# tatsy/normalizing-flows-pytorch

Hardware: AMD Instinct MI355X
Metric: samples/sec (train step: forward flow + log-det + NLL + backward + Adam) (higher is better)
Workload: dtype f32; 1 GPU; Glow CIFAR-shape (3,32,32) L=3 K=32 batch 64 per GPU (512 over 8); per_gpu_batch=64, global_batch=64, parallelism=dp1, hipgraph=True, deterministic=True, dp_one_graph=False

## Files before the change

### normalizing-flows-pytorch_amd/csrc/conv_chain.hip

```cpp
#include <cstdlib>
#include <cstring>
#include <mutex>
#include <unordered_set>
#include "nf_conv_core.h"
#include "nf_det.h"

NF_DET_STATE(nf_ccd)
NF_DET_HOST_API(nf_ccd)
#include "nf_bf16x3.h"
#include "nf_small_plu.h"

#define NF_CC_NL 6
#define NF_CC_NB 5
#define NF_CC_MAX_BLOCKS NF_CONVNET_MAX_BLOCKS

#define NF_CC_WG_SLOTS (NF_CC_NB * NF_CC_MAX_BLOCKS * 64)
#define NF_CC_GROUP 16
#define NF_CC_MAX_GROUPS ((NF_CC_MAX_BLOCKS + NF_CC_GROUP - 1) / NF_CC_GROUP)
#define NF_CC_FLAT_MAX 128
#define NF_CC_STAT_SLOTS (NF_CC_WG_SLOTS + NF_CC_NB * NF_CC_MAX_GROUPS * 64)
static_assert(2 * NF_CC_STAT_SLOTS == NF_CONVNET_WS_FLOATS, "exchange workspace size in include/nfhip.h");

NF_PERSIST_STATE(nf_cc)
NF_PERSIST_HOST_API(nf_cc)
// ... 828 lines not shown
        for (int j = 0; j < 4; ++j) sc[j] = An[64 + min(16 * rt + 4 * lk + j, C - 1)];
        f32x4 acc = (f32x4){0.f, 0.f, 0.f, 0.f};
#pragma unroll
        for (int q = 0; q < KQ; ++q) {
            const int c = 4 * q + lk;
            const float bv = c < C ? gv[q] : 0.f;
            const float a = (ra < C && c < C) ? av[q] : 0.f;
            acc = __builtin_amdgcn_mfma_f32_16x16x4f32(a, bv, acc, 0, 0, 0);
        }
        float* gxb = gx + b * cs.n_full + p;
        const int row = p >> lgWf, xx = p & (cs.W - 1);
#pragma unroll
        for (int j = 0; j < 4; ++j) {
            const int r = 16 * rt + 4 * lk + j;
            const float v = acc[j] * sc[j];
            if (r < C) gxb[(int64_t)r * P] = v;
            int which, m, sp;
            if (cs.mode == NF_SPLIT_CHANNEL) {
                const int hc = C >> 1, sel = r >= hc ? 1 : 0;
                which = sel ^ cs.odd; m = r - sel * hc; sp = p;
            } else {
                const int k = 4 * r + 2 * (row & 1) + (xx & 1);
                const int qd = (k >= C ? 1 : 0) + (k >= 2 * C ? 1 : 0) + (k >= 3 * C ? 1 : 0);
                const int sel = (qd == 1 || qd == 2) ? 1 : 0;
                which = sel ^ cs.odd; m = sel ? k - C : (qd == 0 ? k : k - 2 * C);
                sp = (row >> 1) * cs.w + (xx >> 1);
            }
            if (r < C && which == 0) G0[m * PXW + sidx * HWh + (sp - sp0)] = v;
        }
    };
#pragma unroll
    for (int u = 0; u < 2; ++u) {
        const int item = wid + u * NF_CV_WAVES;
        if (item < nitem && b0 + (item / RT) / per < B) run(item, R.gv[u]);
    }
#pragma unroll 1
    for (int item = wid + 2 * NF_CV_WAVES; item < nitem; item += NF_CV_WAVES) {
        const int blk = item / RT, sidx = blk / per, rem = blk - sidx * per;
        const int64_t b = b0 + sidx;
        if (b >= B) continue;
        const float* gb = d.hd_g_h + b * cs.n_full + fo_lo * cs.W + (rem << 4) + li;
        float gv[KQ];
#pragma unroll
        for (int q = 0; q < KQ; ++q) {
            const int c = 4 * q + lk;
            gv[q] = gb[(int64_t)(c < C ? c : 0) * P];
        }
        run(item, gv);
    }
    NF_CC_STAMP(104);
    asm volatile("s_waitcnt lgkmcnt(0)\n\ts_barrier" ::: "memory");
}
template <int CT>
__device__ __forceinline__ void nf_cc_head_small_bwd(const nf_convnet_bwd_desc& d, const NfSplit& cs, float* hl, int64_t b0, int nsamp,
                                                     int fo_lo, int fo_hi, int64_t B, int PXW, int HWh, int sp0) {
    const int P = cs.H * cs.W, npx = (fo_hi - fo_lo) * cs.W;
    float* const gx = const_cast<float*>(d.cp_g_y);
    float* const G0 = hl + NF_CC_HD_X1;
    const int lgWf = 31 - __clz(cs.W);
    float G[CT];
    int idx = threadIdx.x;
    auto place = [&](int i, int& sidx, int& p, int64_t& base) {
        sidx = i / npx;
        p = fo_lo * cs.W + (i - sidx * npx);
        base = (b0 + sidx) * cs.n_full + p;
    };
    int sidx = 0, p = 0;
    int64_t base = 0;
    bool ok = idx < nsamp * npx;
    if (ok) {
        place(idx, sidx, p, base);
        ok = b0 + sidx < B;
    }
#pragma unroll
    for (int r = 0; r < CT; ++r) G[r] = ok ? d.hd_g_h[base + (int64_t)r * P] : 0.f;
    float Wm[CT][CT], es[CT];
#pragma unroll
    for (int r = 0; r < CT; ++r)
#pragma unroll
        for (int c = 0; c < CT; ++c) Wm[r][c] = d.hd_W[r * CT + c];
#pragma unroll
    for (int c = 0; c < CT; ++c) es[c] = 1.f / expf(d.hd_ls[c]);
    while (idx < nsamp * npx) {
        if (ok) {
            const int row = p >> lgWf, xx = p & (cs.W - 1);
#pragma unroll
            for (int c = 0; c < CT; ++c) {
                float a = 0.f;
#pragma unroll
                for (int r = 0; r < CT; ++r) a = fmaf(Wm[r][c], G[r], a);
                const float v = a * es[c];
                gx[base + (int64_t)c * P] = v;
                int which, m, sp;
                if (cs.mode == NF_SPLIT_CHANNEL) {
                    const int hc = CT >> 1, sel = c >= hc ? 1 : 0;
                    which = sel ^ cs.odd; m = c - sel * hc; sp = p;
                } else {
                    const int k = 4 * c + 2 * (row & 1) + (xx & 1);
                    const int qd = (k >= CT ? 1 : 0) + (k >= 2 * CT ? 1 : 0) + (k >= 3 * CT ? 1 : 0);
                    const int sel = (qd == 1 || qd == 2) ? 1 : 0;
                    which = sel ^ cs.odd; m = sel ? k - CT : (qd == 0 ? k : k - 2 * CT);
                    sp = (row >> 1) * cs.w + (xx >> 1);
                }
                if (which == 0) G0[m * PXW + sidx * HWh + (sp - sp0)] = v;
            }
        }
        idx += NF_CV_THREADS;
        ok = idx < nsamp * npx;
        if (ok) {
            place(idx, sidx, p, base);
            ok = b0 + sidx < B;
        }
#pragma unroll
        for (int r = 0; r < CT; ++r) G[r] = ok ? d.hd_g_h[base + (int64_t)r * P] : 0.f;
    }
    asm volatile("s_waitcnt lgkmcnt(0)\n\ts_barrier" ::: "memory");
}

template <int NPB, int NKQ, bool HALO, bool CPL, int FWc, int CSc, bool PK>
__global__ void __launch_bounds__(NF_CV_THREADS) k_convnet_chain_fwd(nf_convnet_desc d, NfCvGeo g, int I0, int O_out, int training,
                                                                     float eps, float mom, NfSplit cs) {
    static_assert(NPB * NKQ == NF_CV_WAVES, "sixteen waves");
    constexpr int OWN = 16 / NKQ, PXW = 32 * NPB;
    extern __shared__ __attribute__((aligned(16))) float sm[];
    const int OCB = (O_out + 31) / 32;
    const NfCcLds L = nf_cc_lds<NPB, NKQ>(g.CS, OCB);
    float* Wl = sm + L.WL;
    float* RS = sm + L.RS;
    float* kc = sm + L.KC;
    float* kb = sm + L.KB;
    float* red = sm + L.RED;
    const int CSr = FWc > 0 ? CSc : g.CS;
    const int WPs = L.WPs;
    const int lane = threadIdx.x & 63, wid = threadIdx.x >> 6, c32 = lane & 31, hs = lane >> 5;
    const int pb = wid % NPB, kq = wid / NPB;
    const int64_t Npx = g.B * g.HW;
    const int64_t tile = blockIdx.x;
    const int64_t b0 = (tile * PXW) >> g.lgHW;
    constexpr bool halo = HALO;
    const int y0 = halo ? (int)((tile * PXW) & (g.HW - 1)) >> g.lgW : 0;
    unsigned long long* hslots = halo ? (unsigned long long*)d.ws_zero + NF_CC_STAT_SLOTS : nullptr;
    const int px = pb * 32 + c32;
    const int fpos = nf_cv_frame_of(g, px);
    const int64_t P = tile * PXW + px;
    const bool pv = P < Npx;
    const int64_t b = pv ? P >> g.lgHW : 0;
    const int64_t q = pv ? P & (g.HW - 1) : 0;
    const int npb = nf_cc_valid_px(Npx, tile * PXW + 32 * pb, 32);
    unsigned long long* slots = (unsigned long long*)d.ws_zero;
    const unsigned gbase = 8u * (unsigned)d.ws_gen;

    constexpr bool packed = PK;
    constexpr bool cpl = CPL;
    NF_CC_STAMP(0);
#ifdef NF_CC_NO_HEAD_FWD
    const bool headed = false;
#else
    const bool headed = cpl && d.hd_x != nullptr;
#endif
    const int hf = cs.mode == NF_SPLIT_CHECKER ? 2 : 1;
    const int h_ns = halo ? 1 : (g.HW < PXW ? PXW >> g.lgHW : 1);
    const int h_olo = halo ? hf * y0 : 0, h_ohi = halo ? hf * (y0 + g.TH) : cs.H;
    const int h_rlo = halo ? max(h_olo - hf, 0) : 0, h_rhi = halo ? min(h_ohi + hf, cs.H) : cs.H;
    const int h_per = ((h_rhi - h_rlo) * cs.W) >> 4, h_nblk = h_ns * h_per;
    const int h_sp0 = (h_rlo / hf) * g.W, h_np1 = ((h_rhi - h_rlo) / hf) * g.W;
    const bool hsmall = headed && cs.C <= 4;
    NfCcHeadReq hreq;
    if (headed && !hsmall) {
        if (cs.C <= 16) nf_cc_head_request<4>(hreq, d, cs, b0, h_rlo, h_per, h_nblk, g.B);
        else if (cs.C <= 24) nf_cc_head_request<6>(hreq, d, cs, b0, h_rlo, h_per, h_nblk, g.B);
        else if (cs.C <= 48) nf_cc_head_request<12>(hreq, d, cs, b0, h_rlo, h_per, h_nblk, g.B);
        else nf_cc_head_request<16>(hreq, d, cs, b0, h_rlo, h_per, h_nblk, g.B);
    }
    NF_CC_STAMP(105);
    for (int e = threadIdx.x; e < 3 * NF_CC_FP(g.CS); e += NF_CV_THREADS) sm[L.FA + e] = 0.f;
    float* Fr = sm + L.FA;
    NF_CC_STAMP(106);
    if (hsmall) {
        const bool add_ld = !halo || y0 == 0;
        if (cs.C == 3) nf_cc_head_small_fwd<3>(d, cs, RS, b0, h_ns, h_rlo, h_rhi, h_olo, h_ohi, h_sp0, h_np1, g.B, add_ld);
        else if (cs.C == 4) nf_cc_head_small_fwd<4>(d, cs, RS, b0, h_ns, h_rlo, h_rhi, h_olo, h_ohi, h_sp0, h_np1, g.B, add_ld);
        else nf_cc_head_small_fwd<2>(d, cs, RS, b0, h_ns, h_rlo, h_rhi, h_olo, h_ohi, h_sp0, h_np1, g.B, add_ld);
    } else if (headed) {
        const bool add_ld = !halo || y0 == 0;
        if (cs.C <= 16) nf_cc_head_fwd<4>(hreq, d, cs, RS, b0, h_ns, h_rlo, h_olo, h_ohi, h_per, h_nblk, h_sp0, h_np1, g.B, add_ld);
        else if (cs.C <= 24) nf_cc_head_fwd<6>(hreq, d, cs, RS, b0, h_ns, h_rlo, h_olo, h_ohi, h_per, h_nblk, h_sp0, h_np1, g.B, add_ld);
        else if (cs.C <= 48) nf_cc_head_fwd<12>(hreq, d, cs, RS, b0, h_ns, h_rlo, h_olo, h_ohi, h_per, h_nblk, h_sp0, h_np1, g.B, add_ld);
        else nf_cc_head_fwd<16>(hreq, d, cs, RS, b0, h_ns, h_rlo, h_olo, h_ohi, h_per, h_nblk, h_sp0, h_np1, g.B, add_ld);
    }
    NF_CC_STAMP(107);
    if (cpl && !headed) {
        if (!halo) {
            const int nsamp = g.HW < PXW ? PXW >> g.lgHW : 1;
            const int64_t left = g.B - b0;
            const int n4 = (int)(left < nsamp ? (left > 0 ? left : 0) : nsamp) * (cs.n_full >> 2);
            const float4* src = reinterpret_cast<const float4*>(d.cp_z + b0 * cs.n_full);
            float4* dst = reinterpret_cast<float4*>(d.cp_y + b0 * cs.n_full);
            for (int idx = threadIdx.x; idx < n4; idx += NF_CV_THREADS) dst[idx] = src[idx];
        } else if (b0 < g.B) {
            const int plane4 = (cs.H * cs.W) >> 2, chunk4 = (int)(((int64_t)plane4 * PXW) >> g.lgHW);
            const int part = (int)((tile * PXW) & (g.HW - 1)) / PXW;
            const float4* src = reinterpret_cast<const float4*>(d.cp_z + b0 * cs.n_full);
            float4* dst = reinterpret_cast<float4*>(d.cp_y + b0 * cs.n_full);
            for (int idx = threadIdx.x; idx < cs.C * chunk4; idx += NF_CV_THREADS) {
                const int c = idx / chunk4, r = idx - c * chunk4;
                dst[c * plane4 + part * chunk4 + r] = src[c * plane4 + part * chunk4 + r];
            }
        }
    }

    float stream[OWN], own[OWN];
#pragma unroll
    for (int rr = 0; rr < OWN; ++rr) stream[rr] = 0.f;

    f32x16 acc;
#pragma unroll
    for (int r = 0; r < 16; ++r) acc[r] = 0.f;
    {
        const int nchunks = (I0 + 31) / 32;
        const float* in0 = d.x + b0 * I0 * g.HW;
        for (int ch = 0; ch < nchunks; ++ch) {
            const int i0 = 32 * ch, IC = min(32, I0 - i0), ICP = (IC + 7) & ~7, noct = ICP >> 3;
            NfCcW wv;
            if (!packed) nf_cc_w_load<false>(wv, d.w[0], I0, i0, IC, noct);
            __syncthreads();
            if (packed) {
                nf_cc_dma_image(Wl, d.wpk[0] + (size_t)ch * NF_CONV_PACK_IMAGE_FLOATS, wid, lane);
            } else {
                nf_cc_w_store<false>(wv, Wl, WPs, noct);
                if ((9 * noct) & 1) nf_cc_w_zero_slot(Wl, WPs, 9 * noct);
            }
            for (int item = threadIdx.x; item < noct * g.FSZ; item += NF_CV_THREADS) {
                const int o = item / g.FSZ, f = item - o * g.FSZ;
                const int t = nf_cv_decode(g, b0, y0, f);
                const int sp = t >= 0 ? NF_CV_SP(t) : 0, sg_ = t >= 0 ? NF_CV_SEG(t) : 0;
                float v[8];
                if (headed) {
                    const float* X1 = RS + NF_CC_HD_X1 + (sg_ * I0 + i0 + 8 * o) * h_np1 + (sp - h_sp0);
#pragma unroll
                    for (int j = 0; j < 8; ++j) v[j] = (t >= 0 && 8 * o + j < IC) ? X1[j * h_np1] : 0.f;
                } else {
#pragma unroll
                    for (int j = 0; j < 8; ++j) v[j] = (t >= 0 && 8 * o + j < IC) ? in0[(sg_ * I0 + i0 + 8 * o + j) * g.HW + sp] : 0.f;
                }
                nf_cc_frame_store8(Fr, CSr, o, f, v);
            }
            if (packed) nf_cc_dma_wait();
            __syncthreads();
            if (FWc > 0 && ICP == 32) nf_cc_kloop_level<FWc, CSc, NKQ>(acc, Wl, Fr, fpos, c32, hs, kq);
            else {
                int p0, np;
                nf_cc_pair_range((9 * noct + 1) >> 1, NKQ, kq, p0, np);
                nf_cc_kloop<9>(acc, Wl, Fr, WPs, CSr, g.FW, noct, fpos, c32, hs, p0, np);
            }
        }
    }

    NF_CC_STAMP(1);
    float nb_ = 0.f, ng_ = 0.f, nbe_ = 0.f;
    if (threadIdx.x < 32) { nb_ = d.b[0][threadIdx.x]; ng_ = d.gamma[0][threadIdx.x]; nbe_ = d.beta[0][threadIdx.x]; }
#pragma unroll 1
    for (int l = 0; l < NF_CC_NB; ++l) {
        constexpr bool PREFETCH_W = OWN <= 4;
        NfCcW wv;
        if (!packed && PREFETCH_W && l < NF_CC_NB - 1) nf_cc_w_load<false>(wv, d.w[l + 1], 32, 0, 32, 4);
        if (threadIdx.x < 32) { kb[threadIdx.x] = nb_; kb[32 + threadIdx.x] = ng_; kb[64 + threadIdx.x] = nbe_; }
        __syncthreads();
        if (packed && (l < NF_CC_NB - 1 || cpl)) nf_cc_dma_image(Wl, d.wpk[l + 1], wid, lane);
        NF_CC_STAMP(2 + 8 * l);
        nf_cc_ksplit_exchange<NKQ>(own, acc, RS, pb, kq, lane);
        NF_CC_STAMP(3 + 8 * l);
        float* act = d.acts[l];
#pragma unroll
        for (int rr = 0; rr < OWN; ++rr) own[rr] = pv ? own[rr] + (((l & 1) == 0 && l > 0) ? stream[rr] : 0.f) : 0.f;
        if (training) {
            float S, M2;
            int which;
            nf_cc_half_stats<OWN>(own, npb > 0, npb > 16, c32, S, M2, which);
            if (c32 < OWN) {
                const int oc = nf_cv_cd_row(OWN * kq + which, hs);
                red[pb * 32 + oc] = S;
                red[NPB * 32 + pb * 32 + oc] = M2;
            }
        }
#pragma unroll
        for (int rr = 0; rr < OWN; ++rr) {
            const int oc = nf_cv_cd_row(OWN * kq + rr, hs);
            const float a = own[rr] + kb[oc];
            own[rr] = a;
            if (pv) act[(b * 32 + oc) * g.HW + q] = a;
            if ((l & 1) == 0) stream[rr] = a;
        }
        if (halo) nf_cc_halo_publish<OWN>(hslots, gbase, l, g, (int)tile, y0, px, kq, hs, own);
        NF_CC_STAMP(4 + 8 * l);
        unsigned long long hw[2] = {0ull, 0ull};
        if (training) {
            int k;
            float tS, tM2;
            const bool fin = nf_cc_stats_exchange<NPB>(sm, L, slots, gbase, l, Npx, PXW, k, tS, tM2, [&] {
                if (halo) nf_cc_halo_peek(hw, hslots, l, g, (int)tile, y0);
            });
            NF_CC_STAMP(5 + 8 * l);
            if (fin) {
                const float invN = 1.f / (float)Npx;
                const float mean = kb[k] + tS * invN;
                const float var = tM2 * invN;
                const float invstd = 1.f / sqrtf(var + eps);
                const float sc = kb[32 + k] * invstd;
                kc[k] = sc;
                kc[32 + k] = kb[64 + k] - mean * sc;
                if (blockIdx.x == 0) {
                    d.save_mean[l][k] = mean;
                    d.save_invstd[l][k] = invstd;
                    const float unb = Npx > 1 ? var * ((float)Npx / (float)(Npx - 1)) : var;
                    d.rmean[l][k] = (1.f - mom) * d.rmean[l][k] + mom * mean;
                    d.rvar[l][k] = (1.f - mom) * d.rvar[l][k] + mom * unb;
                    if (k == 0 && d.nbt[l] != nullptr) d.nbt[l][0] += 1;
                }
            }
        } else {
            __syncthreads();
            if (threadIdx.x < 32) {
                const int k = threadIdx.x;
                const float mean = d.rmean[l][k], invstd = 1.f / sqrtf(d.rvar[l][k] + eps);
                const float sc = kb[32 + k] * invstd;
                kc[k] = sc;
                kc[32 + k] = kb[64 + k] - mean * sc;
                if (blockIdx.x == 0) {
                    d.save_mean[l][k] = mean;
                    d.save_invstd[l][k] = invstd;
                }
            }
        }
        __syncthreads();
        NF_CC_STAMP(6 + 8 * l);
#pragma unroll
        for (int j = 0; j < OWN / 4; ++j) {
            const int c0 = nf_cv_cd_row(OWN * kq + 4 * j, hs);
            float4 v;
            v.x = pv ? fmaxf(fmaf(own[4 * j + 0], kc[c0 + 0], kc[32 + c0 + 0]), 0.f) : 0.f;
            v.y = pv ? fmaxf(fmaf(own[4 * j + 1], kc[c0 + 1], kc[32 + c0 + 1]), 0.f) : 0.f;
            v.z = pv ? fmaxf(fmaf(own[4 * j + 2], kc[c0 + 2], kc[32 + c0 + 2]), 0.f) : 0.f;
            v.w = pv ? fmaxf(fmaf(own[4 * j + 3], kc[c0 + 3], kc[32 + c0 + 3]), 0.f) : 0.f;
            nf_cc_frame_store4(Fr, CSr, c0, fpos, v.x, v.y, v.z, v.w);
        }
        if constexpr (OWN == 1) {
            const int c0 = nf_cv_cd_row(kq, hs);
            nf_cc_frame_store1(Fr, CSr, c0, fpos, pv ? fmaxf(fmaf(own[0], kc[c0], kc[32 + c0]), 0.f) : 0.f);
        }
        if constexpr (OWN == 2) {
            const int c0 = nf_cv_cd_row(OWN * kq, hs);
            nf_cc_frame_store2(Fr, CSr, c0, fpos, pv ? fmaxf(fmaf(own[0], kc[c0], kc[32 + c0]), 0.f) : 0.f,
                               pv ? fmaxf(fmaf(own[1], kc[c0 + 1], kc[32 + c0 + 1]), 0.f) : 0.f);
        }
        if (halo && threadIdx.x < 32 * g.W) {
            const int c = threadIdx.x >> g.lgW;
#pragma unroll
            for (int s2 = 0; s2 < 2; ++s2) {
                float v = 0.f;
                const int f = nf_cc_halo_poll(hslots, gbase, l, g, (int)tile, y0, s2, v, hw[s2]);
                if (f >= 0) nf_cc_frame_store1(Fr, CSr, c, f, fmaxf(fmaf(v, kc[c], kc[32 + c]), 0.f));
            }
        }
        if (l < NF_CC_NB - 1) {
            if (threadIdx.x < 32) { nb_ = d.b[l + 1][threadIdx.x]; ng_ = d.gamma[l + 1][threadIdx.x]; nbe_ = d.beta[l + 1][threadIdx.x]; }
            if (!packed) {
                if (!PREFETCH_W) nf_cc_w_load<false>(wv, d.w[l + 1], 32, 0, 32, 4);
                nf_cc_w_store<false>(wv, Wl, WPs, 4);
            } else {
                nf_cc_dma_wait();
            }
            __syncthreads();
            NF_CC_STAMP(7 + 8 * l);
#pragma unroll
            for (int r = 0; r < 16; ++r) acc[r] = 0.f;
            if (FWc > 0) nf_cc_kloop_level<FWc, CSc, NKQ>(acc, Wl, Fr, fpos, c32, hs, kq);
            else {
                int p0, np;
                nf_cc_pair_range(18, NKQ, kq, p0, np);
                asm volatile("" : "+s"(np));
                nf_cc_kloop<9>(acc, Wl, Fr, WPs, CSr, g.FW, 4, fpos, c32, hs, p0, np);
            }
            NF_CC_STAMP(8 + 8 * l);
        }
    }
    NF_CC_STAMP(50);

    const int Ch = O_out >> 1;
    const bool packed5 = packed && cpl;
    if (packed5) nf_cc_dma_wait();
    for (int e = threadIdx.x; e < (packed5 ? 0 : 32 * OCB * 4); e += NF_CV_THREADS) {
        const int row = e >> 2, o = e & 3;
        int oc = row;
        if (cpl) {
            const int m = 16 * (row >> 5) + ((row & 31) >> 1);
            oc = (row & 1) ? Ch + m : m;
            if (m >= Ch) oc = O_out;
        }
        float v[8];
        const float4 lo = oc < O_out ? *(const float4*)(d.w[5] + oc * 32 + 8 * o) : make_float4(0.f, 0.f, 0.f, 0.f);
        const float4 hi = oc < O_out ? *(const float4*)(d.w[5] + oc * 32 + 8 * o + 4) : make_float4(0.f, 0.f, 0.f, 0.f);
        v[0] = lo.x; v[1] = lo.y; v[2] = lo.z; v[3] = lo.w; v[4] = hi.x; v[5] = hi.y; v[6] = hi.z; v[7] = hi.w;
        nf_cc_w_put8(Wl, WPs, 4 * (row >> 5) + o, row & 31, v);
    }
    __syncthreads();
    float ls = 0.f;
    const float ca = cpl ? d.cp_a[0] : 0.f, cc = cpl ? d.cp_c[0] : 0.f;
    const int lgw = cpl ? 31 - __clz(cs.w) : 0;
    for (int ob = kq; ob < OCB; ob += NKQ) {
        f32x16 a5;
#pragma unroll
        for (int r = 0; r < 16; ++r) a5[r] = 0.f;
        nf_cc_kloop<1>(a5, Wl + 4 * ob * NF_CC_WSLOT, Fr, WPs, CSr, g.FW, 4, fpos, c32, hs, 0, 2);
        if (!cpl) {
#pragma unroll
            for (int r = 0; r < 16; ++r) {
                const int oc = ob * 32 + nf_cv_cd_row(r, hs);
                if (pv && oc < O_out) d.out[(b * O_out + oc) * g.HW + q] = a5[r] + d.b[5][oc];
            }
        } else {
#pragma unroll
            for (int r = 0; r < 16; r += 2) {
                const int m = 16 * ob + (nf_cv_cd_row(r, hs) >> 1);
                if (pv && m < Ch) {
                    const float t = a5[r] + d.b[5][m], sr = a5[r + 1] + d.b[5][Ch + m];
                    const float th = tanhf(sr), sv = th * ca + cc;
                    const float es = expf(d.cp_inverse ? -sv : sv);
                    d.out[(b * O_out + m) * g.HW + q] = es;
                    d.out[(b * O_out + Ch + m) * g.HW + q] = th;
                    const int64_t o = b * cs.n_full + nf_cc_half_to_full(cs, 0, m, (int)q, lgw);
                    const float z0 = d.cp_z[o];
                    d.cp_y[o] = d.cp_inverse ? es * (z0 - t) : z0 * es + t;
                    ls += sv;
                }
            }
        }
    }
    if (cpl) {
        __syncthreads();
        RS[(kq * 2 + hs) * PXW + px] = ls;
        __syncthreads();
        if (threadIdx.x < PXW) {
            float v = 0.f;
#pragma unroll
            for (int k = 0; k < 2 * NKQ; ++k) v += RS[k * PXW + threadIdx.x];
            const int seg = g.HW < NF_WAVE ? g.HW : NF_WAVE;
            for (int off = seg >> 1; off > 0; off >>= 1) v += __shfl_xor(v, off, NF_WAVE);
            if (g.HW <= NF_WAVE) {
                const int64_t bb = b0 + ((int)threadIdx.x >> g.lgHW);
                if ((threadIdx.x & (g.HW - 1)) == 0 && bb < g.B) atomicAdd(d.cp_ld + bb, d.cp_inverse ? -v : v);
            } else if (lane == 0) {
                red[wid] = v;
            }
        }
        if (g.HW > NF_WAVE) {
            __syncthreads();
            if (threadIdx.x == 0 && b0 < g.B) {
                float v = 0.f;
                for (int k = 0; k < (min(g.HW, PXW) >> 6); ++k) v += red[k];
                if (halo) {
                    const int nparts = g.HW / PXW, part = (int)((tile * PXW) & (g.HW - 1)) / PXW;
                    unsigned long long* hs0 = hslots + (size_t)(tile - part) * NF_CC_HALO_SLOTS(g.W);
                    const unsigned long long gen = (unsigned long long)(gbase + 7u) << 32;
                    if (part > 0) {
                        __hip_atomic_store(hs0 + part, gen | (unsigned long long)__float_as_uint(v), __ATOMIC_RELAXED, __HIP_MEMORY_SCOPE_AGENT);
                        v = 0.f;
                    } else {
                        for (int p2 = 1; p2 < nparts; ++p2) {
                            unsigned long long w;
                            unsigned spins = 0;
                            do {
                                w = __hip_atomic_load(hs0 + p2, __ATOMIC_RELAXED, __HIP_MEMORY_SCOPE_AGENT);
                                if ((unsigned)(w >> 32) == gbase + 7u) break;
                                if (++spins > nf_cc_spin_limit) { NF_PERSIST_GIVE_UP(nf_cc); break; }
                                __builtin_amdgcn_s_sleep(1);
                            } while (true);
                            v += __uint_as_float((unsigned)w);
                        }
                    }
                    if (part == 0) atomicAdd(d.cp_ld + b0, d.cp_inverse ? -v : v);
                } else {
                    atomicAdd(d.cp_ld + b0, d.cp_inverse ? -v : v);
                }
            }
        }
    }
    NF_CC_STAMP(51);
}

template <int OWN>
__device__ __forceinline__ void nf_cc_half_sums2(const float (&u)[OWN], const float (&v)[OWN], int c32, float& S1, float& S2, int& which) {
    static_assert(OWN == 1 || OWN == 2 || OWN == 4 || OWN == 8, "16 / NKQ values per lane");
    if constexpr (OWN == 1) {
        S1 = u[0];
        S2 = v[0];
        for (int m = 1; m < 32; m *= 2) {
            S1 += nf_cc_xor(S1, m);
            S2 += nf_cc_xor(S2, m);
        }
        which = 0;
        return;
    }
    if constexpr (OWN == 2) {
        const bool up = c32 & 1;
        S1 = (up ? u[1] : u[0]) + __shfl_xor(up ? u[0] : u[1], 1, NF_WAVE);
        S2 = (up ? v[1] : v[0]) + __shfl_xor(up ? v[0] : v[1], 1, NF_WAVE);
        for (int m = 2; m < 32; m *= 2) {
            S1 += __shfl_xor(S1, m, NF_WAVE);
            S2 += __shfl_xor(S2, m, NF_WAVE);
        }
        which = up ? 1 : 0;
        return;
    }
    float a4[4], b4[4];
    int w = 0, m = 1;
    if (OWN == 8) {
        const bool up = c32 & 1;
#pragma unroll
        for (int k = 0; k < 4; ++k) {
            a4[k] = (up ? u[k + 4] : u[k]) + nf_cc_xor(up ? u[k] : u[k + 4], 1);
            b4[k] = (up ? v[k + 4] : v[k]) + nf_cc_xor(up ? v[k] : v[k + 4], 1);
        }
        w = up ? 4 : 0;
        m = 2;
    } else {
#pragma unroll
        for (int k = 0; k < 4; ++k) { a4[k] = u[k]; b4[k] = v[k]; }
    }
    float a2[2], b2[2];
    {
        const bool up = c32 & m;
#pragma unroll
        for (int k = 0; k < 2; ++k) {
            a2[k] = (up ? a4[k + 2] : a4[k]) + nf_cc_xor(up ? a4[k] : a4[k + 2], m);
            b2[k] = (up ? b4[k + 2] : b4[k]) + nf_cc_xor(up ? b4[k] : b4[k + 2], m);
        }
        w += up ? 2 : 0;
        m *= 2;
    }
    {
        const bool up = c32 & m;
        S1 = (up ? a2[1] : a2[0]) + nf_cc_xor(up ? a2[0] : a2[1], m);
        S2 = (up ? b2[1] : b2[0]) + nf_cc_xor(up ? b2[0] : b2[1], m);
        w += up ? 1 : 0;
        m *= 2;
    }
    for (; m < 32; m *= 2) {
        S1 += nf_cc_xor(S1, m);
        S2 += nf_cc_xor(S2, m);
    }
    which = w;
}

template <int NPB, typename Peek>
__device__ __forceinline__ const float* nf_cc_sum_exchange(float* sm, const NfCcLds& L, unsigned long long* slots, unsigned gbase, int round,
                                                           Peek&& peek) {
    float* red = sm + L.RED;
    float* xs = sm + L.RS;
    float* tot = sm + L.TOT;
    const int G = gridDim.x;
    __syncthreads();
    if (threadIdx.x < 64) {
        const int i = threadIdx.x & 31, h = threadIdx.x >> 5;
        float sv[NPB];
#pragma unroll
        for (int q = 0; q < NPB; ++q) sv[q] = red[(h * NPB + q) * 32 + i];
#pragma unroll
        for (int w = 1; w < NPB; w *= 2)
#pragma unroll
            for (int q = 0; q < NPB; q += 2 * w) sv[q] += sv[q + w];
        if (G == 1) tot[threadIdx.x] = sv[0];
        else
            __hip_atomic_store(slots + ((size_t)round * NF_CC_MAX_BLOCKS + blockIdx.x) * 64 + threadIdx.x,
                               ((unsigned long long)(gbase + round + 1) << 32) | (unsigned long long)__float_as_uint(sv[0]), __ATOMIC_RELAXED,
                               __HIP_MEMORY_SCOPE_AGENT);
    }
    if (G == 1) {
        peek();
        __syncthreads();
        return tot;
    }
    const int XS = 65;
    const unsigned gen = gbase + (unsigned)(round + 1);
    const unsigned long long* rs = slots + (size_t)round * NF_CC_MAX_BLOCKS * 64;
    const int lane = threadIdx.x & 63, ci = 2 * (threadIdx.x >> 6) + (lane >> 5), l = lane & 31;
    int nrows = G;
    if (NF_CC_MAX_BLOCKS > NF_CC_FLAT_MAX && G > NF_CC_FLAT_MAX) {
        const int grp = blockIdx.x / NF_CC_GROUP;
        unsigned long long* gs = slots + NF_CC_WG_SLOTS + (size_t)round * NF_CC_MAX_GROUPS * 64;
        if (blockIdx.x % NF_CC_GROUP == 0) {
            const int nmem = min(NF_CC_GROUP, G - grp * NF_CC_GROUP);
            nf_cc_collect_slots(xs, rs + (size_t)grp * NF_CC_GROUP * 64, gen, nmem, XS);
            __syncthreads();
            float pa = 0.f, pb = 0.f;
            for (int b = l; b < nmem; b += 32) { pa += xs[b * XS + ci]; pb += xs[b * XS + 32 + ci]; }
            const float A = nf_cc_sum32(pa), Bs = nf_cc_sum32(pb);
            if (l == 0) {
                __hip_atomic_store(gs + grp * 64 + ci, ((unsigned long long)gen << 32) | (unsigned long long)__float_as_uint(A),
                                   __ATOMIC_RELAXED, __HIP_MEMORY_SCOPE_AGENT);
                __hip_atomic_store(gs + grp * 64 + 32 + ci, ((unsigned long long)gen << 32) | (unsigned long long)__float_as_uint(Bs),
                                   __ATOMIC_RELAXED, __HIP_MEMORY_SCOPE_AGENT);
            }
            __syncthreads();
        }
        rs = gs;
        nrows = (G + NF_CC_GROUP - 1) / NF_CC_GROUP;
    }
    nf_cc_collect_slots(xs, rs, gen, nrows, XS);
    peek();
    __syncthreads();
    {
        float pa = 0.f, pb = 0.f;
        for (int b = l; b < nrows; b += 32) { pa += xs[b * XS + ci]; pb += xs[b * XS + 32 + ci]; }
        const float A = nf_cc_sum32(pa), Bs = nf_cc_sum32(pb);
        if (l == 0) { tot[ci] = A; tot[32 + ci] = Bs; }
    }
    __syncthreads();
    return tot;
}

template <int NPB, int NKQ, bool HALO, bool CPL, int FWc, int CSc, bool PK>
__global__ void __launch_bounds__(NF_CV_THREADS) k_convnet_chain_bwd(nf_convnet_bwd_desc d, NfCvGeo g, int I0, int O_out, int training,
                                                                     NfSplit cs) {
    static_assert(NPB * NKQ == NF_CV_WAVES, "sixteen waves");
    constexpr int OWN = 16 / NKQ, PXW = 32 * NPB;
    extern __shared__ __attribute__((aligned(16))) float sm[];
    const NfCcLds L = nf_cc_lds<NPB, NKQ>(g.CS, 1);
    float* Wl = sm + L.WL;
    float* RS = sm + L.RS;
    float* kc = sm + L.KC;
    float* red = sm + L.RED;
    const int CSr = FWc > 0 ? CSc : g.CS;
    const int WPs = L.WPs;
    const int lane = threadIdx.x & 63, wid = threadIdx.x >> 6, c32 = lane & 31, hs = lane >> 5;
    const int pb = wid % NPB, kq = wid / NPB;
    const int64_t Npx = g.B * g.HW;
    const int64_t tile = blockIdx.x;
    const int px = pb * 32 + c32;
    const int fpos = nf_cv_frame_of(g, px);
    const int64_t P = tile * PXW + px;
    const bool pv = P < Npx;
    const int64_t b = pv ? P >> g.lgHW : 0;
    const int64_t q = pv ? P & (g.HW - 1) : 0;
    const float invN = 1.f / (float)Npx;
    unsigned long long* slots = (unsigned long long*)d.ws_zero;
    const unsigned gbase = 8u * (unsigned)d.ws_gen;
    const int64_t b0 = (tile * PXW) >> g.lgHW;
    constexpr bool halo = HALO;
    const int y0 = halo ? (int)((tile * PXW) & (g.HW - 1)) >> g.lgW : 0;
    unsigned long long* hslots = halo ? slots + NF_CC_STAT_SLOTS : nullptr;
    float gstream_h[2] = {0.f, 0.f};

    NF_CC_STAMP(64);
    const bool hbw = CPL && d.hd_g_h != nullptr;
    const int hb_hf = cs.mode == NF_SPLIT_CHECKER ? 2 : 1;
    const int hb_ns = halo ? 1 : (g.HW < PXW ? PXW >> g.lgHW : 1);
    const int hb_lo = halo ? hb_hf * y0 : 0, hb_hi = halo ? hb_hf * (y0 + g.TH) : cs.H;
    const int hb_per = ((hb_hi - hb_lo) * cs.W) >> 4, hb_nblk = hb_ns * hb_per;
    NfCcHeadBwdReq hbreq;
    const bool hbs = hbw && cs.C <= 4;
    if (hbw && !hbs) {
        if (cs.C <= 16) nf_cc_head_bwd_request<4>(hbreq, d, cs, b0, hb_lo, hb_per, hb_nblk, g.B);
        else if (cs.C <= 24) nf_cc_head_bwd_request<6>(hbreq, d, cs, b0, hb_lo, hb_per, hb_nblk, g.B);
        else if (cs.C <= 48) nf_cc_head_bwd_request<12>(hbreq, d, cs, b0, hb_lo, hb_per, hb_nblk, g.B);
        else nf_cc_head_bwd_request<16>(hbreq, d, cs, b0, hb_lo, hb_per, hb_nblk, g.B);
    }
    for (int e = threadIdx.x; e < 3 * NF_CC_FP(g.CS); e += NF_CV_THREADS) sm[L.FA + e] = 0.f;
    float* Fr = sm + L.FA;
    const bool bnv = L.BNV >= 0;
    constexpr bool packed = PK;
    const int nch0 = (I0 + 31) / 32;
    if (packed) nf_cc_dma_image(Wl, d.wpk[5] + NF_CONV_PACK_IMAGE_FLOATS, wid, lane);
    if (bnv && threadIdx.x < NF_CC_NB * 128) {
        const int l2 = threadIdx.x >> 7, j = (threadIdx.x >> 5) & 3, k = threadIdx.x & 31;
        const float* src = j == 0 ? d.save_mean[l2] : (j == 1 ? d.save_invstd[l2] : (j == 2 ? d.gamma[l2] : d.beta[l2]));
        sm[L.BNV + threadIdx.x] = src[k];
    }

    constexpr bool cpl = CPL;
    NF_CC_STAMP(100);
    if (hbs) {
        const int hb_sp0 = halo ? y0 * g.W : 0;
        if (cs.C == 3) nf_cc_head_small_bwd<3>(d, cs, RS, b0, hb_ns, hb_lo, hb_hi, g.B, PXW, g.HW, hb_sp0);
        else if (cs.C == 4) nf_cc_head_small_bwd<4>(d, cs, RS, b0, hb_ns, hb_lo, hb_hi, g.B, PXW, g.HW, hb_sp0);
        else nf_cc_head_small_bwd<2>(d, cs, RS, b0, hb_ns, hb_lo, hb_hi, g.B, PXW, g.HW, hb_sp0);
    } else if (hbw) {
        const int hb_sp0 = halo ? y0 * g.W : 0;
        if (cs.C <= 16) nf_cc_head_bwd<4>(hbreq, d, cs, RS, b0, hb_lo, hb_per, hb_nblk, g.B, PXW, g.HW, hb_sp0);
        else if (cs.C <= 24) nf_cc_head_bwd<6>(hbreq, d, cs, RS, b0, hb_lo, hb_per, hb_nblk, g.B, PXW, g.HW, hb_sp0);
        else if (cs.C <= 48) nf_cc_head_bwd<12>(hbreq, d, cs, RS, b0, hb_lo, hb_per, hb_nblk, g.B, PXW, g.HW, hb_sp0);
        else nf_cc_head_bwd<16>(hbreq, d, cs, RS, b0, hb_lo, hb_per, hb_nblk, g.B, PXW, g.HW, hb_sp0);
    }
    NF_CC_STAMP(101);
    const int Ch = O_out >> 1;
    const int lgw = cpl ? 31 - __clz(cs.w) : 0;
    const float ca = cpl ? d.cp_a[0] : 0.f;
    float acc_a = 0.f, acc_c = 0.f;
    f32x16 acc;
#pragma unroll
    for (int r = 0; r < 16; ++r) acc[r] = 0.f;
    {
        const int npair = (O_out + 15) >> 4;
        if (packed) nf_cc_dma_wait();
        for (int e = threadIdx.x; e < (packed ? 0 : npair * 2 * 32); e += NF_CV_THREADS) {
            const int o = e >> 5, ic = e & 31;
            float v[8];
#pragma unroll
            for (int j = 0; j < 8; ++j) v[j] = 8 * o + j < O_out ? d.w[5][(8 * o + j) * 32 + ic] : 0.f;
            nf_cc_w_put8(Wl, WPs, o, ic, v);
        }
        __syncthreads();
        int p0, np;
        nf_cc_pair_range(npair, NKQ, kq, p0, np);
        const float* go = cpl ? nullptr : d.g_out + b * O_out * g.HW + q;
        const float gl = (cpl && pv) ? d.cp_g_ld[b] : 0.f;
#pragma unroll 1
        for (int pi = p0; pi < p0 + np; ++pi) {
            float bv[8];
#pragma unroll
            for (int j = 0; j < 8; ++j) {
                const int oc = 16 * pi + 8 * hs + j;
                const bool ok = pv && oc < O_out;
                float v = 0.f;
                if (!cpl) {
                    v = ok ? go[(int64_t)oc * g.HW] : 0.f;
                } else if (ok) {
                    const bool is_s = oc >= Ch;
                    const int m = is_s ? oc - Ch : oc;
                    const int64_t o = b * cs.n_full + nf_cc_half_to_full(cs, 0, m, (int)q, lgw);
                    const float gy0 = hbw ? RS[NF_CC_HD_X1 + m * PXW + px] : d.cp_g_y[o];
                    v = gy0;
                    if (is_s) {
                        const float th = d.cp_out[(b * O_out + oc) * g.HW + q];
                        const float es = d.cp_out[(b * O_out + m) * g.HW + q];
                        d.cp_g_z[o] = gy0 * es;
                        const float gs = gy0 * d.cp_z[o] * es + gl;
                        v = gs * ca * (1.f - th * th);
                        acc_a += gs * th;
                        acc_c += gs;
                    }
                    d.cp_g_out[(b * O_out + oc) * g.HW + q] = v;
                }
                bv[j] = v;
            }
            bf16x8 bh, bm, bl;
#pragma unroll
            for (int j = 0; j < 8; j += 2) {
                bf16x2 h2, m2, l2;
                nf_cc_split2(f32x2{bv[j], bv[j + 1]}, h2, m2, l2);
                bh[j] = h2[0]; bh[j + 1] = h2[1];
                bm[j] = m2[0]; bm[j + 1] = m2[1];
                bl[j] = l2[0]; bl[j + 1] = l2[1];
            }
            const float* wa = Wl + (2 * pi + hs) * NF_CC_WSLOT + 4 * c32;
            const bf16x8 ah = *(const bf16x8*)(wa), am = *(const bf16x8*)(wa + WPs), al = *(const bf16x8*)(wa + 2 * WPs);
            NF_CC_MFMA6(ah, am, al, bh, bm, bl);
        }
        if (cpl) {
#pragma unroll
            for (int off = 32; off > 0; off >>= 1) {
                acc_a += __shfl_xor(acc_a, off, NF_WAVE);
                acc_c += __shfl_xor(acc_c, off, NF_WAVE);
            }
            if (lane == 0) { red[wid] = acc_a; red[NF_CV_WAVES + wid] = acc_c; }
        }
    }

    float gstream[OWN], own[OWN];
#pragma unroll
    for (int rr = 0; rr < OWN; ++rr) gstream[rr] = 0.f;
    NF_CC_STAMP(65);

#pragma unroll 1
    for (int l = NF_CC_NB - 1; l >= 0; --l) {
        if (threadIdx.x < 32) {
            const int k = threadIdx.x;
            const float* v = sm + L.BNV + 128 * l;
            const float mean = bnv ? v[k] : d.save_mean[l][k], invstd = bnv ? v[32 + k] : d.save_invstd[l][k];
            const float sc = (bnv ? v[64 + k] : d.gamma[l][k]) * invstd;
            kc[k] = sc;
            kc[32 + k] = (bnv ? v[96 + k] : d.beta[l][k]) - mean * sc;
            kc[64 + k] = mean;
            kc[96 + k] = invstd;
        }
        float xh[OWN];
        {
            const float* act = d.acts[l];
#pragma unroll
            for (int rr = 0; rr < OWN; ++rr) {
                const int oc = nf_cv_cd_row(OWN * kq + rr, hs);
                xh[rr] = pv ? act[(b * 32 + oc) * g.HW + q] : 0.f;
            }
        }
        float a_h[2] = {0.f, 0.f};
        if (halo && threadIdx.x < 32 * g.W) {
            const int c = threadIdx.x >> g.lgW, x = threadIdx.x & (g.W - 1);
            if (y0 > 0) a_h[0] = d.acts[l][(b0 * 32 + c) * g.HW + (y0 - 1) * g.W + x];
            if (y0 + g.TH < g.H) a_h[1] = d.acts[l][(b0 * 32 + c) * g.HW + (y0 + g.TH) * g.W + x];
        }
        __syncthreads();
        if (packed) {
            if (l >= 1) nf_cc_dma_image(Wl, d.wpk[l] + NF_CONV_PACK_IMAGE_FLOATS, wid, lane);
            else if (d.g_x != nullptr || cpl) nf_cc_dma_image(Wl, d.wpk[0] + (size_t)nch0 * NF_CONV_PACK_IMAGE_FLOATS, wid, lane);
        }
        NF_CC_STAMP(66 + 6 * (4 - l));
        if (cpl && l == NF_CC_NB - 1 && threadIdx.x == 0) {
            float ta = 0.f, tc = 0.f;
            for (int k = 0; k < NF_CV_WAVES; ++k) { ta += red[k]; tc += red[NF_CV_WAVES + k]; }
            if (nf_det_on(nf_ccd_det)) {
                const float v2[2] = {ta, tc};
                float* const dst2[2] = {d.cp_g_a, d.cp_g_c};
                if (!nf_det_fold_add<2>(nf_ccd_det_slab, nf_ccd_det_cnt, v2, dst2)) {
                    nf_det_wait(nf_ccd_det);
                    atomicAdd(d.cp_g_a, ta);
                    atomicAdd(d.cp_g_c, tc);
                    nf_det_pass(nf_ccd_det);
                }
            } else {
                atomicAdd(d.cp_g_a, ta);
                atomicAdd(d.cp_g_c, tc);
            }
        }
        nf_cc_ksplit_exchange<NKQ>(own, acc, RS, pb, kq, lane);
        NF_CC_STAMP(67 + 6 * (4 - l));
        float* gn = d.gn[l];
#pragma unroll
        for (int rr = 0; rr < OWN; ++rr) {
            const int oc = nf_cv_cd_row(OWN * kq + rr, hs);
            const float a = xh[rr];
            const bool keep = pv && fmaf(a, kc[oc], kc[32 + oc]) > 0.f;
            const float v = keep ? own[rr] : 0.f;
            own[rr] = v;
            xh[rr] = (a - kc[64 + oc]) * kc[96 + oc];
            if (pv) gn[(b * 32 + oc) * g.HW + q] = v;
        }
        if (halo) nf_cc_halo_publish<OWN>(hslots, gbase, l, g, (int)tile, y0, px, kq, hs, own);
        float mg[OWN], mgx[OWN];
        unsigned long long hw[2] = {0ull, 0ull};
        const float* tot;
        {
            float p2[OWN], S1, S2;
            int which;
#pragma unroll
            for (int rr = 0; rr < OWN; ++rr) p2[rr] = own[rr] * xh[rr];
            nf_cc_half_sums2<OWN>(own, p2, c32, S1, S2, which);
            if (c32 < OWN) {
                const int oc = nf_cv_cd_row(OWN * kq + which, hs);
                red[pb * 32 + oc] = S1;
                red[NPB * 32 + pb * 32 + oc] = S2;
            }
            tot = nf_cc_sum_exchange<NPB>(sm, L, slots, gbase, l, [&] {
                if (halo) nf_cc_halo_peek(hw, hslots, l, g, (int)tile, y0);
            });
            NF_CC_STAMP(68 + 6 * (4 - l));
            if (blockIdx.x == 0 && threadIdx.x < 64) {
                (threadIdx.x < 32 ? d.sum_g[l] : d.sum_gx[l])[threadIdx.x & 31] = tot[threadIdx.x];
                float* sink = threadIdx.x < 32 ? d.g_beta[l] : d.g_gamma[l];
                if (sink != nullptr) sink[threadIdx.x & 31] += tot[threadIdx.x];
            }
#pragma unroll
            for (int rr = 0; rr < OWN; ++rr) {
                const int oc = nf_cv_cd_row(OWN * kq + rr, hs);
                mg[rr] = training ? tot[oc] * invN : 0.f;
                mgx[rr] = training ? tot[32 + oc] * invN : 0.f;
            }
        }
        const bool on_stream = (l & 1) == 0;
        float* gs = (l == 4) ? d.g_store[0] : (l == 2 ? d.g_store[1] : nullptr);
#pragma unroll
        for (int rr = 0; rr < OWN; ++rr) {
            const int oc = nf_cv_cd_row(OWN * kq + rr, hs);
            float G = kc[oc] * (own[rr] - mg[rr] - xh[rr] * mgx[rr]);
            if (on_stream) G += gstream[rr];
            G = pv ? G : 0.f;
            own[rr] = G;
            if (on_stream) gstream[rr] = G;
            if (gs != nullptr && pv) gs[(b * 32 + oc) * g.HW + q] = G;
        }
#pragma unroll
        for (int j = 0; j < OWN / 4; ++j) {
            const int c0 = nf_cv_cd_row(OWN * kq + 4 * j, hs);
            nf_cc_frame_store4(Fr, CSr, c0, fpos, own[4 * j], own[4 * j + 1], own[4 * j + 2], own[4 * j + 3]);
        }
        if constexpr (OWN == 2) nf_cc_frame_store2(Fr, CSr, nf_cv_cd_row(OWN * kq, hs), fpos, own[0], own[1]);
        if constexpr (OWN == 1) nf_cc_frame_store1(Fr, CSr, nf_cv_cd_row(kq, hs), fpos, own[0]);
        if (halo && threadIdx.x < 32 * g.W) {
            const int c = threadIdx.x >> g.lgW;
            const float mgc = training ? tot[c] * invN : 0.f, mgxc = training ? tot[32 + c] * invN : 0.f;
#pragma unroll
            for (int s2 = 0; s2 < 2; ++s2) {
                float v = 0.f;
                const int f = nf_cc_halo_poll(hslots, gbase, l, g, (int)tile, y0, s2, v, hw[s2]);
                if (f >= 0) {
                    const float xhh = (a_h[s2] - kc[64 + c]) * kc[96 + c];
                    float G = kc[c] * (v - mgc - xhh * mgxc);
                    if ((l & 1) == 0) { G += gstream_h[s2]; gstream_h[s2] = G; }
// ... 387 lines not shown
```

Baseline: 3209 samples/s.

## Prefetch BN params into LDS via async DMA and batch coupling loads

Result: faster. 3307 samples/s (median of 6 runs) (+3.0%).

```diff
diff --git a/normalizing-flows-pytorch_amd/csrc/conv_chain.hip b/normalizing-flows-pytorch_amd/csrc/conv_chain.hip
--- a/normalizing-flows-pytorch_amd/csrc/conv_chain.hip
+++ b/normalizing-flows-pytorch_amd/csrc/conv_chain.hip
@@ -1004,6 +1004,7 @@
 
     constexpr bool packed = PK;
     constexpr bool cpl = CPL;
+    constexpr bool kb_dma = !HALO && NPB != 8;
     NF_CC_STAMP(0);
 #ifdef NF_CC_NO_HEAD_FWD
     const bool headed = false;
@@ -1041,6 +1042,23 @@
         else nf_cc_head_fwd<16>(hreq, d, cs, RS, b0, h_ns, h_rlo, h_olo, h_ohi, h_per, h_nblk, h_sp0, h_np1, g.B, add_ld);
     }
     NF_CC_STAMP(107);
+    if (kb_dma && wid == 0) {
+        __builtin_amdgcn_global_load_lds((const __attribute__((address_space(1))) void*)((hs ? d.gamma[0] : d.b[0]) + c32),
+                                         (__attribute__((address_space(3))) void*)kb, 4, 0, 0);
+        if (!hs)
+            __builtin_amdgcn_global_load_lds((const __attribute__((address_space(1))) void*)(d.beta[0] + c32),
+                                             (__attribute__((address_space(3))) void*)(kb + 64), 4, 0, 0);
+    }
+    const bool rsv = L.BNV >= 0;
+    if (rsv && wid < NF_CC_NB && (blockIdx.x == 0 || !training))
+        __builtin_amdgcn_global_load_lds((const __attribute__((address_space(1))) void*)((hs ? d.rvar[wid] : d.rmean[wid]) + c32),
+                                         (__attribute__((address_space(3))) void*)(sm + L.BNV + 64 * wid), 4, 0, 0);
+    if (rsv && wid >= NF_CC_NB && wid < NF_CC_NB + 3 && 64 * (wid - NF_CC_NB) + hs * 32 + c32 < O_out)
+        __builtin_amdgcn_global_load_lds((const __attribute__((address_space(1))) void*)(d.b[5] + 64 * (wid - NF_CC_NB) + hs * 32 + c32),
+                                         (__attribute__((address_space(3))) void*)(sm + L.BNV + 64 * wid), 4, 0, 0);
+    if (cpl && rsv && wid == NF_CC_NB + 3 && !hs && c32 < 2)
+        __builtin_amdgcn_global_load_lds((const __attribute__((address_space(1))) void*)(c32 ? d.cp_c : d.cp_a),
+                                         (__attribute__((address_space(3))) void*)(sm + L.BNV + 64 * wid), 4, 0, 0);
     if (cpl && !headed) {
         if (!halo) {
             const int nsamp = g.HW < PXW ? PXW >> g.lgHW : 1;
@@ -1110,13 +1128,15 @@
 
     NF_CC_STAMP(1);
     float nb_ = 0.f, ng_ = 0.f, nbe_ = 0.f;
-    if (threadIdx.x < 32) { nb_ = d.b[0][threadIdx.x]; ng_ = d.gamma[0][threadIdx.x]; nbe_ = d.beta[0][threadIdx.x]; }
+    if (!kb_dma && threadIdx.x < 32) { nb_ = d.b[0][threadIdx.x]; ng_ = d.gamma[0][threadIdx.x]; nbe_ = d.beta[0][threadIdx.x]; }
 #pragma unroll 1
     for (int l = 0; l < NF_CC_NB; ++l) {
         constexpr bool PREFETCH_W = OWN <= 4;
         NfCcW wv;
+        if (!packed && l == 0) nf_cc_dma_wait();
         if (!packed && PREFETCH_W && l < NF_CC_NB - 1) nf_cc_w_load<false>(wv, d.w[l + 1], 32, 0, 32, 4);
-        if (threadIdx.x < 32) { kb[threadIdx.x] = nb_; kb[32 + threadIdx.x] = ng_; kb[64 + threadIdx.x] = nbe_; }
+        if ((!kb_dma || l > 0) && threadIdx.x < 32) { kb[threadIdx.x] = nb_; kb[32 + threadIdx.x] = ng_; kb[64 + threadIdx.x] = nbe_; }
+        if (kb_dma && packed && l == 0) nf_cc_dma_wait();
         __syncthreads();
         if (packed && (l < NF_CC_NB - 1 || cpl)) nf_cc_dma_image(Wl, d.wpk[l + 1], wid, lane);
         NF_CC_STAMP(2 + 8 * l);
@@ -1165,16 +1185,18 @@
                     d.save_mean[l][k] = mean;
                     d.save_invstd[l][k] = invstd;
                     const float unb = Npx > 1 ? var * ((float)Npx / (float)(Npx - 1)) : var;
-                    d.rmean[l][k] = (1.f - mom) * d.rmean[l][k] + mom * mean;
-                    d.rvar[l][k] = (1.f - mom) * d.rvar[l][k] + mom * unb;
-                    if (k == 0 && d.nbt[l] != nullptr) d.nbt[l][0] += 1;
+                    const float rm_ = rsv ? sm[L.BNV + 64 * l + k] : d.rmean[l][k], rv_ = rsv ? sm[L.BNV + 64 * l + 32 + k] : d.rvar[l][k];
+                    d.rmean[l][k] = (1.f - mom) * rm_ + mom * mean;
+                    d.rvar[l][k] = (1.f - mom) * rv_ + mom * unb;
+                    if (k == 0 && d.nbt[l] != nullptr) atomicAdd((unsigned long long*)d.nbt[l], 1ull);
                 }
             }
         } else {
             __syncthreads();
             if (threadIdx.x < 32) {
                 const int k = threadIdx.x;
-                const float mean = d.rmean[l][k], invstd = 1.f / sqrtf(d.rvar[l][k] + eps);
+                const float mean = rsv ? sm[L.BNV + 64 * l + k] : d.rmean[l][k];
+                const float invstd = 1.f / sqrtf((rsv ? sm[L.BNV + 64 * l + 32 + k] : d.rvar[l][k]) + eps);
                 const float sc = kb[32 + k] * invstd;
                 kc[k] = sc;
                 kc[32 + k] = kb[64 + k] - mean * sc;
@@ -1255,39 +1277,68 @@
         v[0] = lo.x; v[1] = lo.y; v[2] = lo.z; v[3] = lo.w; v[4] = hi.x; v[5] = hi.y; v[6] = hi.z; v[7] = hi.w;
         nf_cc_w_put8(Wl, WPs, 4 * (row >> 5) + o, row & 31, v);
     }
+    const float* b5 = rsv ? sm + L.BNV + 64 * NF_CC_NB : RS;
+    if (!rsv && (int)threadIdx.x < O_out) RS[threadIdx.x] = d.b[5][threadIdx.x];
     __syncthreads();
     float ls = 0.f;
-    const float ca = cpl ? d.cp_a[0] : 0.f, cc = cpl ? d.cp_c[0] : 0.f;
+    const float ca = cpl ? (rsv ? sm[L.BNV + 64 * (NF_CC_NB + 3)] : d.cp_a[0]) : 0.f;
+    const float cc = cpl ? (rsv ? sm[L.BNV + 64 * (NF_CC_NB + 3) + 1] : d.cp_c[0]) : 0.f;
     const int lgw = cpl ? 31 - __clz(cs.w) : 0;
+    int qe = (int)q, be = pv ? (int)(b - b0) : 0, hse = hs, c32e = c32, fpe = fpos;
+    asm volatile("" : "+v"(qe), "+v"(be), "+v"(hse), "+v"(c32e), "+v"(fpe));
+    const unsigned sb = (unsigned)be;
+    const char* zs = cpl ? (const char*)(d.cp_z + b0 * cs.n_full) : nullptr;
+    char* ys = cpl ? (char*)(d.cp_y + b0 * cs.n_full) : nullptr;
+    float* os = d.out + b0 * O_out * g.HW;
+    const unsigned vo = 4u * ((sb * (unsigned)O_out + 2u * hse) * (unsigned)g.HW + (unsigned)qe);
+    auto zoff = [&](int m) { return 4u * (sb * (unsigned)cs.n_full + (unsigned)nf_cc_half_to_full(cs, 0, m, qe, lgw)); };
+    constexpr int ZB = 8;
+    float z0[ZB];
+    auto request_z0 = [&](int ob, int j0) {
+#pragma unroll
+        for (int jj = 0; jj < ZB; ++jj) {
+            const int m = 16 * ob + (nf_cv_cd_row(2 * (j0 + jj), hse) >> 1);
+            const bool ok = pv && m < Ch;
+            z0[jj] = ok ? *(const float*)(zs + zoff(m)) : 0.f;
+        }
+    };
+    NF_CC_STAMP(120);
     for (int ob = kq; ob < OCB; ob += NKQ) {
+        if (cpl) request_z0(ob, 0);
         f32x16 a5;
 #pragma unroll
         for (int r = 0; r < 16; ++r) a5[r] = 0.f;
-        nf_cc_kloop<1>(a5, Wl + 4 * ob * NF_CC_WSLOT, Fr, WPs, CSr, g.FW, 4, fpos, c32, hs, 0, 2);
+        nf_cc_kloop<1>(a5, Wl + 4 * ob * NF_CC_WSLOT, Fr, WPs, CSr, g.FW, 4, fpe, c32e, hse, 0, 2);
+        if (ob == kq) NF_CC_STAMP(121);
         if (!cpl) {
 #pragma unroll
             for (int r = 0; r < 16; ++r) {
-                const int oc = ob * 32 + nf_cv_cd_row(r, hs);
-                if (pv && oc < O_out) d.out[(b * O_out + oc) * g.HW + q] = a5[r] + d.b[5][oc];
+                const int oc = ob * 32 + nf_cv_cd_row(r, hse);
+                if (pv && oc < O_out) os[((int64_t)be * O_out + oc) * g.HW + qe] = a5[r] + b5[oc];
             }
         } else {
 #pragma unroll
-            for (int r = 0; r < 16; r += 2) {
-                const int m = 16 * ob + (nf_cv_cd_row(r, hs) >> 1);
-                if (pv && m < Ch) {
-                    const float t = a5[r] + d.b[5][m], sr = a5[r + 1] + d.b[5][Ch + m];
-                    const float th = tanhf(sr), sv = th * ca + cc;
-                    const float es = expf(d.cp_inverse ? -sv : sv);
-                    d.out[(b * O_out + m) * g.HW + q] = es;
-                    d.out[(b * O_out + Ch + m) * g.HW + q] = th;
-                    const int64_t o = b * cs.n_full + nf_cc_half_to_full(cs, 0, m, (int)q, lgw);
-                    const float z0 = d.cp_z[o];
-                    d.cp_y[o] = d.cp_inverse ? es * (z0 - t) : z0 * es + t;
-                    ls += sv;
+            for (int j0 = 0; j0 < 8; j0 += ZB) {
+                if (j0 > 0) request_z0(ob, j0);
+#pragma unroll
+                for (int jj = 0; jj < ZB; ++jj) {
+                    const int r = 2 * (j0 + jj);
+                    const int mr = 16 * ob + (nf_cv_cd_row(r, 0) >> 1), m = mr + 2 * hse;
+                    if (pv && m < Ch) {
+                        const float t = a5[r] + b5[m], sr = a5[r + 1] + b5[Ch + m];
+                        const float th = tanhf(sr), sv = th * ca + cc;
+                        const float es = expf(d.cp_inverse ? -sv : sv);
+                        const float z = z0[jj];
+                        *(float*)((char*)(os + (int64_t)mr * g.HW) + vo) = es;
+                        *(float*)((char*)(os + (int64_t)(Ch + mr) * g.HW) + vo) = th;
+                        *(float*)(ys + zoff(m)) = d.cp_inverse ? es * (z - t) : z * es + t;
+                        ls += sv;
+                    }
                 }
             }
         }
     }
+    NF_CC_STAMP(122);
     if (cpl) {
         __syncthreads();
         RS[(kq * 2 + hs) * PXW + px] = ls;
@@ -1530,6 +1581,7 @@
     }
 
     constexpr bool cpl = CPL;
+    constexpr int BZ = 8;
     NF_CC_STAMP(100);
     if (hbs) {
         const int hb_sp0 = halo ? y0 * g.W : 0;
@@ -1547,6 +1599,7 @@
     const int Ch = O_out >> 1;
     const int lgw = cpl ? 31 - __clz(cs.w) : 0;
     const float ca = cpl ? d.cp_a[0] : 0.f;
+    const float gl = (cpl && pv) ? d.cp_g_ld[b] : 0.f;
     float acc_a = 0.f, acc_c = 0.f;
     f32x16 acc;
 #pragma unroll
@@ -1565,35 +1618,64 @@
         int p0, np;
         nf_cc_pair_range(npair, NKQ, kq, p0, np);
         const float* go = cpl ? nullptr : d.g_out + b * O_out * g.HW + q;
-        const float gl = (cpl && pv) ? d.cp_g_ld[b] : 0.f;
+        const unsigned sb = pv ? (unsigned)(b - b0) : 0u;
+        const unsigned vo = 4u * ((sb * (unsigned)O_out + 8u * hs) * (unsigned)g.HW + (unsigned)q);
+        const float* co = cpl ? d.cp_out + b0 * O_out * g.HW : nullptr;
+        float* cgo = cpl ? d.cp_g_out + b0 * O_out * g.HW : nullptr;
+        const char* zs = cpl ? (const char*)(d.cp_z + b0 * cs.n_full) : nullptr;
+        const char* gys = cpl ? (const char*)(d.cp_g_y + b0 * cs.n_full) : nullptr;
+        char* gzs = cpl ? (char*)(d.cp_g_z + b0 * cs.n_full) : nullptr;
+        auto zoff = [&](int m) { return 4u * (sb * (unsigned)cs.n_full + (unsigned)nf_cc_half_to_full(cs, 0, m, (int)q, lgw)); };
+        NF_CC_STAMP(123);
 #pragma unroll 1
         for (int pi = p0; pi < p0 + np; ++pi) {
             float bv[8];
-#pragma unroll
-            for (int j = 0; j < 8; ++j) {
-                const int oc = 16 * pi + 8 * hs + j;
-                const bool ok = pv && oc < O_out;
-                float v = 0.f;
-                if (!cpl) {
-                    v = ok ? go[(int64_t)oc * g.HW] : 0.f;
-                } else if (ok) {
-                    const bool is_s = oc >= Ch;
-                    const int m = is_s ? oc - Ch : oc;
-                    const int64_t o = b * cs.n_full + nf_cc_half_to_full(cs, 0, m, (int)q, lgw);
-                    const float gy0 = hbw ? RS[NF_CC_HD_X1 + m * PXW + px] : d.cp_g_y[o];
-                    v = gy0;
-                    if (is_s) {
-                        const float th = d.cp_out[(b * O_out + oc) * g.HW + q];
-                        const float es = d.cp_out[(b * O_out + m) * g.HW + q];
-                        d.cp_g_z[o] = gy0 * es;
-                        const float gs = gy0 * d.cp_z[o] * es + gl;
-                        v = gs * ca * (1.f - th * th);
-                        acc_a += gs * th;
-                        acc_c += gs;
+            if (!cpl) {
+#pragma unroll
+                for (int j = 0; j < 8; ++j) {
+                    const int oc = 16 * pi + 8 * hs + j;
+                    bv[j] = (pv && oc < O_out) ? go[(int64_t)oc * g.HW] : 0.f;
+                }
+            } else {
+                float gy[BZ], th[BZ], es[BZ], zz[BZ];
+#pragma unroll
+                for (int j0 = 0; j0 < 8; j0 += BZ) {
+#pragma unroll
+                    for (int jj = 0; jj < BZ; ++jj) {
+                        const int j = j0 + jj;
+                        const int ocr = 16 * pi + j, oc = ocr + 8 * hs;
+                        const bool ok = pv && oc < O_out, is_s = ok && oc >= Ch;
+                        const int m = oc >= Ch ? oc - Ch : oc;
+                        const unsigned zo = ok ? zoff(m) : 0u;
+                        gy[jj] = ok ? (hbw ? RS[NF_CC_HD_X1 + m * PXW + px] : *(const float*)(gys + zo)) : 0.f;
+                        th[jj] = is_s ? *(const float*)((const char*)(co + (int64_t)ocr * g.HW) + vo) : 0.f;
+                        es[jj] = is_s ? *(const float*)((const char*)(co + (int64_t)(ocr - Ch) * g.HW) + vo) : 0.f;
+                        zz[jj] = is_s ? *(const float*)(zs + zo) : 0.f;
                     }
-                    d.cp_g_out[(b * O_out + oc) * g.HW + q] = v;
+                    if (pi == p0 && j0 == 0) NF_CC_STAMP(124);
+#pragma unroll
+                    for (int jj = 0; jj < BZ; ++jj) {
+                        const int j = j0 + jj;
+                        const int ocr = 16 * pi + j, oc = ocr + 8 * hs;
+                        const bool ok = pv && oc < O_out;
+                        float v = 0.f;
+                        if (ok) {
+                            const bool is_s = oc >= Ch;
+                            const float gy0 = gy[jj];
+                            v = gy0;
+                            if (is_s) {
+                                *(float*)(gzs + zoff(oc - Ch)) = gy0 * es[jj];
+                                const float gs = gy0 * zz[jj] * es[jj] + gl;
+                                v = gs * ca * (1.f - th[jj] * th[jj]);
+                                acc_a += gs * th[jj];
+                                acc_c += gs;
+                            }
+                            *(float*)((char*)(cgo + (int64_t)ocr * g.HW) + vo) = v;
+                        }
+                        bv[j] = v;
+                    }
                 }
-                bv[j] = v;
+                if (pi == p0) NF_CC_STAMP(125);
             }
             bf16x8 bh, bm, bl;
 #pragma unroll
```
